# YiwenShaoStephen/mergeNet

Measured on AMD Instinct MI355X. Metric: merged Mpixels/sec at 1024x2048 (speculative fast path; proven path: value_proven_path), higher is better.
Workload: dtype f32

## Files before the change

mergenet_amd/csrc/mergenet_hip.hip:

```cpp
#include <hip/hip_runtime.h>
#include <hip/hip_ext.h>

#include <math.h>
#include <stdio.h>
#include <stdlib.h>
#include <string.h>
#include <time.h>

#include "../../include/mergenet_hip.h"
#include "mn_device.h"
#include "mn_kernels_score.h"
#include "mn_kernels_merge.h"
#include "mn_kernels_finish.h"
#include "mn_kernels_output.h"
#include "mn_kernels_prepare.h"
#include "mn_kernels_cc.h"
#include "mn_kernels_tail.h"
#include "mn_kernels_exact.h"
#include "mn_kernels_reforder.h"

#define MN_NSCALARS 16
#define MN_STAT_BYTES ((((sizeof(Counters) + 15) & ~(size_t)15)) + MN_NSCALARS * sizeof(int) + 4 * sizeof(double))

#define MN_MAX_SUBROUNDS 64
// ... 552 lines not shown
  S.lpvalid = c->lpvalid;
  return S;
}

template <bool FIRST>
static void launch_edge_pass(mn_context* c, const ImgParams& P, hipStream_t st, u64* out, int s) {
  const int* progress = c->progress;
  const dim3 g(grid_for(P.N, 256)), b(256);
  const dim3 gx(8 * ((grid_for(P.N, 256) + 7) / 8));
  const unsigned char* cls0 = c->ocls;
  const unsigned char* matched = c->matched;
  const bool fast = P.omf > 0.0f && P.sdb == 0.0f && !(c->debug_flags & 1);
  if (fast && P.O == 10 && !P.clip)
    hipLaunchKernelGGL((mn_edge_pass_fast<10, FIRST, false>), gx, b, 0, st, P, cls0, matched, out,
                       progress, s);
  else if (fast && P.O == 10)
    hipLaunchKernelGGL((mn_edge_pass_fast<10, FIRST, true>), gx, b, 0, st, P, cls0, matched, out,
                       progress, s);
  else if (fast && P.O == 16 && !P.clip)
    hipLaunchKernelGGL((mn_edge_pass_fast<16, FIRST, false>), gx, b, 0, st, P, cls0, matched, out,
                       progress, s);
  else if (fast && P.O == 16)
    hipLaunchKernelGGL((mn_edge_pass_fast<16, FIRST, true>), gx, b, 0, st, P, cls0, matched, out,
                       progress, s);
  else
    hipLaunchKernelGGL(mn_edge_pass_generic<FIRST>, g, b, 0, st, P, obj_state(c), matched, out, progress, s);
}

static int run_phase_a(mn_context* c, const ImgParams& P, hipStream_t st, bool edge,
                       FillList* fills = nullptr, bool components = false) {
  const int N = P.N;
  FillList own;
  if (!fills) fills = &own;
  if (!components) {
    fills->add(c->lpvalid, N, 0);
    fills->add(c->matched, N, 0);
  }
  fills->launch(st);
  if (components) {
    if (!c->ext_events) MN_HIP(hipEventRecord(c->ev[0], st));
    return MN_OK;
  }
  hipLaunchKernelGGL(mn_init_objects, dim3(grid_for(N, 256)), dim3(256), 0, st, N, c->osize,
                     c->parent, c->mate);
  MN_HIP(hipEventRecord(c->ev[0], st));
  {
    const unsigned blocks = grid_for((size_t)(N >> 2) > 0 ? (size_t)(N >> 2) : 1, 256);
    hipLaunchKernelGGL(mn_class_pass, dim3(blocks), dim3(256), 0, st, P, c->ocls);
  }
  MN_HIP(hipEventRecord(c->ev[1], st));
  if (edge) {
    launch_edge_pass<true>(c, P, st, c->ball, 0);
  }
  MN_HIP(hipEventRecord(c->ev[2], st));
  MN_HIP(hipMemcpyAsync(c->cls0, c->ocls, N, hipMemcpyDeviceToDevice, st));
  MN_HIP(hipGetLastError());
  return MN_OK;
}

static int read_counters(mn_context* c, hipStream_t st) {
  MN_HIP(hipMemcpyAsync(c->h_cnt, c->cnt, sizeof(Counters), hipMemcpyDeviceToHost, st));
  MN_HIP(hipStreamSynchronize(st));
  return MN_OK;
}

static int build_list(mn_context* c, const ImgParams& P, hipStream_t st, size_t cap, RecList L,
                      bool from_pixels, RecList src, int Rsrc, int* Rout, bool fresh_all = false) {
  ObjState S = obj_state(c);
  HashTab T = c->T;
  T.mask = (unsigned)(cap - 1);
  FillList f;
  f.add(T.key, cap * sizeof(u64), 0xFF);
  f.add(T.S, cap * sizeof(i64), 0);
  f.add(T.touched, cap, 0);
  f.add(&c->cnt->n_records, sizeof(int), 0);
  f.add(c->ball, (size_t)P.N * sizeof(u64), 0);
  f.add(c->gmax, 64 * sizeof(unsigned), 0);
  f.launch(st);
  if (from_pixels)
    hipLaunchKernelGGL(mn_build_from_pixels, dim3(grid_for(P.N, 256)), dim3(256), 0, st, P, S, T);
  else
    hipLaunchKernelGGL(mn_rebuild, dim3(grid_for(Rsrc, MN_REBUILD_ITEMS)), dim3(256), 0, st, S, src,
                       Rsrc, (const unsigned char*)c->matched, T, L, c->ball, c->gmax, c->cnt, fresh_all ? 1 : 0);
  if (cap <= (1u << 16))
    hipLaunchKernelGGL(mn_compact<1>, dim3(grid_for(cap, 256)), dim3(256), 0, st, P, S, T, L,
                       c->ball, c->gmax, c->cnt, (const int*)nullptr, (int*)nullptr);
  else
    hipLaunchKernelGGL(mn_compact<4>, dim3(grid_for(cap, MN_COMPACT_SLOTS)), dim3(256), 0, st, P, S, T, L,
                       c->ball, c->gmax, c->cnt, (const int*)nullptr, (int*)nullptr);
  MN_HIP(hipGetLastError());
  if (read_counters(c, st) != MN_OK) return MN_ERR_NO_DEVICE;
  *Rout = c->h_cnt->n_records;
  return MN_OK;
}

static size_t gsum_stride(int N) {
#ifdef MN_GSUM_SKEW
  return ((((size_t)N / 4 + 63) / 64) | 1) * 64;
#else
  return (size_t)N;
#endif
}

template <int PX>
static void launch_cc_px(mn_context* c, const ImgParams& P, hipStream_t st, unsigned kmask, bool hook,
                         bool cls = false, const unsigned* hook_bits = nullptr,
                         hipEvent_t hook_done = nullptr, bool lean_cls = false) {
  const int N = P.N, ngroups = (N + PX - 1) / PX;
  if (!hook) {
    const dim3 g(grid_for(ngroups, MN_CC_SIGN_THREADS)), b(MN_CC_SIGN_THREADS);
    ClsOut CO;
    CO.ocls = lean_cls ? nullptr : c->ocls; CO.cls0 = c->cls0; CO.lpvalid = lean_cls ? nullptr : c->lpvalid;
    CO.gsum = reinterpret_cast<int*>(c->lpsum);
    CO.gstride = gsum_stride(P.N);
    const bool plain = !P.clip && P.sdb == 0.0f;
#define MN_LAUNCH_SIGN(PLAINV, CLSV)                                                                    \
    do {                                                                                                \
      if (c->ext_events)                                                                                \
        hipExtLaunchKernelGGL((mn_cc_sign<PX, PLAINV, (CLSV) && PX == 4>), g, b, 0, st, c->ev[0], c->ev[10], 0, \
                              P, c->cc_bits, c->cc_negbits, c->scalars + 6, c->partial, CO); \
      else                                                                                              \
        hipLaunchKernelGGL((mn_cc_sign<PX, PLAINV, (CLSV) && PX == 4>), g, b, 0, st, P, c->cc_bits, c->cc_negbits, \
                           c->scalars + 6, c->partial, CO);                                             \
    } while (0)
    if (plain && cls) MN_LAUNCH_SIGN(true, true);
    else if (plain) MN_LAUNCH_SIGN(true, false);
    else if (cls) MN_LAUNCH_SIGN(false, true);
    else MN_LAUNCH_SIGN(false, false);
#undef MN_LAUNCH_SIGN
  } else {
    const dim3 gx(8 * ((grid_for(ngroups, 256) + 7) / 8));
    if (hook_done)
      hipExtLaunchKernelGGL(mn_cc_hook<PX>, gx, dim3(256), 0, st, nullptr, hook_done, 0, P,
                            hook_bits ? hook_bits : (const unsigned*)c->cc_bits, c->parent, kmask);
    else
      hipLaunchKernelGGL(mn_cc_hook<PX>, gx, dim3(256), 0, st, P, hook_bits ? hook_bits : (const unsigned*)c->cc_bits,
                         c->parent, kmask);
  }
}

static int run_components(mn_context* c, const ImgParams& P, hipStream_t& st, bool wait, bool with_ball,
                          bool with_compact, bool fork_before_sums, bool cores = false) {
  const int N = P.N;
  ObjState S = obj_state(c);
  const dim3 b(256);
  const bool four = P.W % 4 == 0;
  int kh = -1, kv = -1, dv = 0;
  for (int k = 0; k < P.O; k++) {
    if (kh < 0 && P.di[k] == 0 && P.dj[k] == 1) kh = k;
    if (kv < 0 && P.dj[k] == 0 && (P.di[k] == 1 || P.di[k] == -1)) { kv = k; dv = P.di[k]; }
  }
  const bool few_events = (c->debug_flags & 2) != 0;
  const bool lean = (c->debug_flags & 16) != 0;
  const dim3 tiles((P.W + 63) / 64, (P.H + MN_CC_TILE_ROWS - 1) / MN_CC_TILE_ROWS);
  const bool sweep4 = (N & 3) == 0 && P.W >= 4;
  const size_t sign_blocks = grid_for((size_t)(sweep4 ? N / 4 : N), MN_CC_SIGN_THREADS);
  c->cc_sign_blocks = (int)(sign_blocks * (MN_CC_SIGN_THREADS / 64));
  int* clsmin = c->root;
  int* clsmax = c->mapbuf;
  const bool fused_cls = sweep4;
  const bool lean_cls = fused_cls && !cores;
  if (sweep4) launch_cc_px<4>(c, P, st, 0u, false, fused_cls, nullptr, nullptr, lean_cls);
  else launch_cc_px<1>(c, P, st, 0u, false);
  if (!few_events && !c->ext_events) MN_HIP(hipEventRecord(c->ev[10], st));
  const unsigned* lbits = c->cc_bits;
  unsigned kshort = 0u;
  if (cores) {
    if (!fused_cls) {
      const unsigned blocks = grid_for((size_t)(N >> 2) > 0 ? (size_t)(N >> 2) : 1, 256);
      hipLaunchKernelGGL(mn_class_pass, dim3(blocks), dim3(256), 0, st, P, c->cls0);
    }
    unsigned* bits2 = reinterpret_cast<unsigned*>(c->label);
    for (int k = 0; k < P.O; k++)
      if (c->core_radius < 0 || (abs(P.di[k]) <= c->core_radius && abs(P.dj[k]) <= c->core_radius)) kshort |= 1u << k;
    hipLaunchKernelGGL(mn_core_clean, dim3(grid_for(N, 256)), b, 0, st, P, (const unsigned*)c->cc_bits,
                       (const unsigned char*)c->cls0, c->pruned, kshort);
    hipLaunchKernelGGL(mn_core_bits, dim3(grid_for(N, 256)), b, 0, st, P, (const unsigned char*)c->pruned,
                       (const unsigned*)c->cc_bits, (const unsigned char*)c->cls0, bits2);
    lbits = bits2;
  }
  hipStream_t real = st;
  if (c->replay.capturing) {
    MN_HIP(hipStreamBeginCapture(c->replay.cap, hipStreamCaptureModeThreadLocal));
    st = c->replay.cap;
  }
  unsigned kmask = P.O >= 32 ? 0xFFFFFFFFu : ((1u << P.O) - 1u);
  const bool fork_ext = fork_before_sums && c->ext_events && !c->replay.capturing;
  bool fork_by_hook = false;
  hipLaunchKernelGGL(mn_cc_tiles, tiles, dim3(MN_CC_TILE_ROWS * 64), 0, st, P, lbits, c->parent, kh, kv, dv,
                     c->osize, c->lp_acc, clsmin, clsmax, c->matched);
  if (kh >= 0 || kv >= 0) {
    hipLaunchKernelGGL(mn_cc_borders, tiles, dim3(128), 0, st, P, lbits, c->parent, kh, kv, dv);
    if (kh >= 0) kmask &= ~(1u << kh);
    if (kv >= 0) kmask &= ~(1u << kv);
  }
  hipLaunchKernelGGL(mn_cc_flatten, dim3(grid_for((size_t)(N >> 2) > 0 ? (size_t)(N >> 2) : 1, 256)), b, 0, st, N, c->parent);
  fork_by_hook = fork_ext && kmask;
  if (kmask) {
    if (four) launch_cc_px<4>(c, P, st, kmask, true, false, lbits, fork_by_hook ? c->ev_fork : nullptr);
    else launch_cc_px<1>(c, P, st, kmask, true, false, lbits, fork_by_hook ? c->ev_fork : nullptr);
  }
  if (c->replay.capturing) {
    MN_HIP(hipStreamEndCapture(c->replay.cap, &c->replay.gA));
    MN_HIP(hipGraphInstantiate(&c->replay.eA, c->replay.gA, nullptr, nullptr, 0));
    MN_HIP(hipGraphLaunch(c->replay.eA, real));
    st = real;
  }
  HashTab T = c->T;
  T.mask = (unsigned)(c->cc_cap - 1);
  if (!few_events && !lean) MN_HIP(hipEventRecord(c->ev[7], st));
  if (fork_before_sums) {
    if (!fork_by_hook) MN_HIP(hipEventRecord(c->ev_fork, st));
    MN_HIP(hipStreamWaitEvent(c->side, c->ev_fork, 0));
    st = c->side;
    if (c->replay.capturing) {
      MN_HIP(hipStreamBeginCapture(c->replay.cap, hipStreamCaptureModeThreadLocal));
      st = c->replay.cap;
    }
  }
  if (!few_events && !lean) MN_HIP(hipEventRecord(c->ev[11], st));
  {
    const size_t lds = (size_t)MN_CC_SUM_SLOTS * (P.C + 1) * sizeof(u64);
    if (lds > c->cc_sum_lds) {
      MN_HIP(hipFuncSetAttribute(reinterpret_cast<const void*>(mn_cc_class_sums),
                                 hipFuncAttributeMaxDynamicSharedMemorySize, (int)lds));
      MN_HIP(hipFuncSetAttribute(reinterpret_cast<const void*>(mn_cc_sums),
                                 hipFuncAttributeMaxDynamicSharedMemorySize, (int)lds));
      c->cc_sum_lds = lds;
    }
    const unsigned blocks = grid_for((size_t)(N >> 2) > 0 ? (size_t)(N >> 2) : 1, MN_CC_SUM_THREADS);
    if (fused_cls)
      hipLaunchKernelGGL(mn_cc_sums, dim3((blocks + MN_CC_SUMS_ITERS - 1) / MN_CC_SUMS_ITERS), dim3(MN_CC_SUM_THREADS), lds, st, P, S,
                         (const unsigned char*)c->cls0, (const int*)reinterpret_cast<int*>(c->lpsum), gsum_stride(P.N),
                         c->lp_acc, clsmin, clsmax, cores ? (const unsigned char*)c->pruned : (const unsigned char*)nullptr);
    else
      hipLaunchKernelGGL(mn_cc_class_sums, dim3(blocks), dim3(MN_CC_SUM_THREADS), lds, st, P, S, c->cls0,
                         c->lp_acc, clsmin, clsmax);
  }
  if (!few_events && !lean) MN_HIP(hipEventRecord(c->ev[8], st));
  if (!cores)
  {
    if (sweep4)
      hipLaunchKernelGGL(mn_cc_cross<4>, dim3((unsigned)grid_for((size_t)N / 4, MN_CC_CROSS_THREADS)), dim3(MN_CC_CROSS_THREADS),
                         0, st, P, (const int*)c->parent, T, (const unsigned*)c->cc_negbits, c->scalars + 6, c->cc_tcount);
    else
      hipLaunchKernelGGL(mn_cc_cross<1>, dim3((unsigned)grid_for((size_t)N, MN_CC_CROSS_THREADS)), dim3(MN_CC_CROSS_THREADS),
                         0, st, P, (const int*)c->parent, T, (const unsigned*)c->cc_negbits, c->scalars + 6, c->cc_tcount);
  }
  if (!few_events && !lean) MN_HIP(hipEventRecord(c->ev[9], st));
  hipLaunchKernelGGL(mn_cc_finish, dim3(grid_for((size_t)(N >> 4) > 0 ? (size_t)(N >> 4) : 1, 256)), b, 0, st, P, S,
                     (const unsigned char*)c->matched, (const i64*)c->lp_acc,
                     (const int*)clsmin, (const int*)clsmax, c->mate, cores ? (int*)nullptr : c->cc_roots,
                     c->scalars + 8, c->scalars + 6, lean_cls ? (const unsigned char*)c->cls0 : (const unsigned char*)nullptr);
  if (cores) {
    const unsigned all = P.O >= 32 ? 0xFFFFFFFFu : ((1u << P.O) - 1u);
    if (kshort != all) {
      MN_HIP(hipMemsetAsync(c->matched, 0, (size_t)N, st));
      hipLaunchKernelGGL(mn_core_check, dim3(grid_for(N, 256)), b, 0, st, P, (const int*)c->parent, lbits, c->matched);
      hipLaunchKernelGGL(mn_core_dissolve, dim3(grid_for(N, 256)), b, 0, st, P, S,
                         (const unsigned char*)c->matched, c->scalars + 9);
    }
    hipLaunchKernelGGL(mn_count_cross_edges, dim3(grid_for(N, 256)), b, 0, st, P, (const int*)c->parent, c->touch);
  }
  if (with_compact)
    hipLaunchKernelGGL(mn_compact<4>, dim3(grid_for(c->cc_cap, MN_COMPACT_SLOTS)), dim3(256), 0, st, P, S,
                       T, c->LA, with_ball ? c->ball : (u64*)nullptr, c->gmax, c->cnt,
                       (const int*)c->cc_tcount, c->cc_lcount);
  MN_HIP(hipGetLastError());
  if (!wait) return 0;
  MN_HIP(hipMemcpyAsync(c->h_scalars, c->scalars, MN_NSCALARS * sizeof(int), hipMemcpyDeviceToHost, st));
  MN_HIP(hipMemcpyAsync(c->h_cnt, c->cnt, sizeof(Counters), hipMemcpyDeviceToHost, st));
  MN_HIP(hipStreamSynchronize(st));
  if (c->h_scalars[6] != 0 || c->h_scalars[7] != 0) {
    MN_HIP(hipMemsetAsync(c->cnt, 0, sizeof(Counters), st));
    return 1;
  }
  return 0;
}

static int exact_setup(mn_context* c, const ImgParams& P, hipStream_t st) {
  int rc = x_ensure(c, P.N, P.O, P.C);
  if (rc != MN_OK) return rc;
  mn_context::XWork& w = c->xw;
  XState& X = w.X;
  const size_t N = (size_t)P.N;
  MN_HIP(hipMemsetAsync(X.hs, 0xFF, (size_t)X.nb * 4 * sizeof(XSlot), st));
  MN_HIP(hipMemsetAsync(X.leaf, 0, (((size_t)X.NB << X.Blog) + 1024) * sizeof(unsigned), st));
  MN_HIP(hipMemsetAsync(X.ostamp, 0, (size_t)N * 2 * sizeof(unsigned), st));
  MN_HIP(hipMemsetAsync(X.freeheads, 0xFF, MN_X_FREE_CLASSES * sizeof(unsigned), st));
  memset(w.h_ctl, 0, sizeof(XCtl));
  w.h_ctl->ttrack = getenv("MN_X_NO_TIE_TRACKING") ? 0 : 1;
  w.h_ctl->bump = 0ull;
  MN_HIP(hipMemcpyAsync(X.ctl, w.h_ctl, sizeof(XCtl), hipMemcpyHostToDevice, st));
  hipLaunchKernelGGL(mn_x_init_objects, dim3(grid_for(N, 256)), dim3(256), 0, st, P, X, c->cls0);
  MN_HIP(hipEventRecord(c->ev[1], st));
  hipLaunchKernelGGL(mn_x_init_records, dim3(grid_for((size_t)X.NL, 256)), dim3(256), 0, st, P, X);
  MN_HIP(hipEventRecord(c->ev[2], st));
  MN_HIP(hipGetLastError());
  return MN_OK;
}

static int exact_loop(mn_context** cs, int n, const ImgParams* Ps, hipStream_t st, unsigned char* full) {
  mn_context::XWork& w0 = cs[0]->xw;
  if (w0.batch_cap < n) {
    if (w0.d_P) (void)hipFree(w0.d_P);
    if (w0.d_X) (void)hipFree(w0.d_X);
    w0.d_P = nullptr; w0.d_X = nullptr;
    MN_HIP(hipMalloc(reinterpret_cast<void**>(&w0.d_P), (size_t)n * sizeof(ImgParams)));
    MN_HIP(hipMalloc(reinterpret_cast<void**>(&w0.d_X), (size_t)n * sizeof(XState)));
    w0.batch_cap = n;
  }
  size_t lds = 0;
  long long max_total = 0;
  {
    XState* hx = static_cast<XState*>(malloc((size_t)n * sizeof(XState)));
    if (!hx) return MN_ERR_INTERNAL;
    for (int i = 0; i < n; i++) {
      const XState& X = cs[i]->xw.X;
      hx[i] = X;
      const size_t l = MN_X_LDS_BYTES(X.NBpad);
      if (l > lds) lds = l;
      const long long mt = 8LL * (long long)X.NL + 65536;
      if (mt > max_total) max_total = mt;
    }
    hipError_t e1 = hipMemcpyAsync(w0.d_P, Ps, (size_t)n * sizeof(ImgParams), hipMemcpyHostToDevice, st);
    hipError_t e2 = hipMemcpyAsync(w0.d_X, hx, (size_t)n * sizeof(XState), hipMemcpyHostToDevice, st);
    hipError_t e3 = hipStreamSynchronize(st);
    free(hx);
    MN_HIP(e1); MN_HIP(e2); MN_HIP(e3);
  }
  if (!w0.lds_ready) {
    MN_HIP(hipFuncSetAttribute(reinterpret_cast<const void*>(mn_x_run),
                               hipFuncAttributeMaxDynamicSharedMemorySize, 160 * 1024));
    w0.lds_ready = 1;
  }
  long long per_launch = 1LL << 24;
  if (const char* e = getenv("MN_X_BUDGET")) { const long long v = atoll(e); if (v > 0) per_launch = v; }
  const long long max_launches = 1 << 20;
  for (long long it = 0; it < max_launches; it++) {
    long long most = 0;
    bool any = false;
    for (int i = 0; i < n; i++) {
      mn_context::XWork& w = cs[i]->xw;
      if (it > 0 && w.h_ctl->status != MN_X_BUDGET) continue;
      any = true;
// ... 1491 lines not shown
```

mergenet_amd/csrc/mn_kernels_cc.h:

```cpp
#pragma once

static_assert(MN_MAX_OFFSETS <= 32, "edge masks are 32-bit words: one bit per offset");

#include "mn_device.h"
#include "mn_kernels_merge.h"

#define MN_LP_FIX 16777216.0

__device__ __forceinline__ int mn_cc_find(int* __restrict__ parent, int x) {
  int p = parent[x];
  while (p != x) {
    const int g = parent[p];
    if (g != p) parent[x] = g;
    x = p;
    p = g;
  }
  return x;
}

struct __attribute__((packed, aligned(4))) mn_int4u { int x, y, z, w; };
__device__ __forceinline__ int4 mn_ld_int4_unaligned(const int* __restrict__ p) {
  const mn_int4u t = *reinterpret_cast<const mn_int4u*>(p);
  return make_int4(t.x, t.y, t.z, t.w);
}
// ... 138 lines not shown
          const float x = (PLAIN || first[g] != INT_MIN) ? mn_cc_value<PLAIN>(P, v[g][j]) : 1.0f;
          m[j] |= (x >= P.sep_hi) ? bit : 0u;
          ng[j] |= (x <= P.sep_lo) ? bit : 0u;
          f *= fmaxf(x, 1.0f - x);
        }
      }
    } else {
#pragma unroll
      for (int g = 0; g < G; g++) {
        const unsigned bit = (k0 + g < P.O) ? (1u << ((k0 + g) & 31)) : 0u;
#pragma unroll
        for (int j = 0; j < PX; j++) {
          const bool second = straddle && c0 + j >= P.W;
          const bool inb = ((rin[g] >> (second ? 1 : 0)) & 1) &&
                           (unsigned)(first[g] + j - (second ? P.W : 0)) < (unsigned)P.W;
          const float x = inb ? mn_cc_value<PLAIN>(P, v[g][j]) : 1.0f;
          inmask[j] |= inb ? bit : 0u;
          m[j] |= (x >= P.sep_hi) ? bit : 0u;
          ng[j] |= (x <= P.sep_lo) ? bit : 0u;
          f *= fmaxf(x, 1.0f - x);
        }
      }
    }
    if (((k0 / G) & 3) == 3 || k0 + G >= P.O) {
      t_sum += (double)logf(f);
      f = 1.0f;
    }
  }
  int bad = 0;
#pragma unroll
  for (int j = 0; j < PX; j++) {
    const unsigned in = fast ? rowmask : inmask[j];
    m[j] &= in;
    ng[j] &= in;
    bad += __popc(in & ~(m[j] | ng[j]));
  }
  if (live) {
    if (PX == 4) {
      mn_st_stream(reinterpret_cast<uint4*>(bits + p0), make_uint4(m[0], m[1 % PX], m[2 % PX], m[3 % PX]));
      mn_st_stream(reinterpret_cast<uint4*>(negbits + p0), make_uint4(ng[0], ng[1 % PX], ng[2 % PX], ng[3 % PX]));
    } else {
      bits[p0] = m[0];
      negbits[p0] = ng[0];
    }
  }
  for (int off = 32; off > 0; off >>= 1) {
    bad += __shfl_xor(bad, off);
    t_sum += __shfl_xor(t_sum, off);
  }
  if (lane == 0) {
    if (bad) atomicAdd(violations, bad);
    const size_t waveg = (size_t)blockIdx.x * (MN_CC_SIGN_THREADS / 64) + wave;
    partial[waveg * 2] = t_sum;
    partial[waveg * 2 + 1] = 0.0;
  }
}

__global__ __launch_bounds__(256) void mn_cc_export_neg(ImgParams P, const unsigned* __restrict__ negbits,
                                                        float* __restrict__ out) {
  const int p = blockIdx.x * 256 + threadIdx.x;
  if (p >= P.N) return;
  unsigned left = negbits[p];
  while (left) {
    const int k = __ffs((int)left) - 1;
    left &= left - 1u;
    const float x = mn_same_value(P, P.same[(size_t)k * P.N + p]);
    out[(size_t)k * P.N + p] = logf(x) - mn_log1m(x);
  }
}

#ifndef MN_CC_TILE_ROWS
#define MN_CC_TILE_ROWS 16
#endif
__global__ __launch_bounds__(MN_CC_TILE_ROWS * 64) void mn_cc_tiles(ImgParams P, const unsigned* __restrict__ bits,
                                                    int* __restrict__ parent, int kh, int kv, int dv,
                                                    int* __restrict__ osize, i64* __restrict__ lp_acc,
                                                    int* __restrict__ clsmin, int* __restrict__ clsmax,
                                                    unsigned char* __restrict__ cand) {
  __shared__ int lab[MN_CC_TILE_ROWS * 64];
  const int t = threadIdx.x, lane = t & 63, i = t >> 6;
  const int r = (int)blockIdx.y * MN_CC_TILE_ROWS + i, c = (int)blockIdx.x * 64 + lane;
  const bool in = r < P.H && c < P.W;
  const int p = in ? r * P.W + c : 0;
  const unsigned b = in ? bits[p] : 0u;
  const bool link = kh >= 0 && ((b >> kh) & 1u) && lane < 63;
  const int ni = i + dv;
  const bool vlink = kv >= 0 && ((b >> kv) & 1u) && ni >= 0 && ni < MN_CC_TILE_ROWS;
  const u64 m = __ballot(link);
  const u64 below = lane ? (~m & ((1ull << lane) - 1ull)) : 0ull;
  const int start = below ? (64 - __clzll((long long)below)) : 0;
  lab[t] = i * 64 + start;
  __syncthreads();
  int a = 0, bb = 0;
  bool want = false;
  if (vlink) {
    a = mn_cc_find(lab, t);
    bb = mn_cc_find(lab, ni * 64 + lane);
    want = a != bb;
  }
  u64 todo = __ballot(want);
  const u64 key = mn_key(a, bb);
  while (todo) {
    const int first = __ffsll((long long)todo) - 1;
    const u64 k0v = ((u64)(unsigned)__shfl((int)(key >> 32), first) << 32) |
                    (u64)(unsigned)__shfl((int)(key & 0xFFFFFFFFull), first);
    const bool mine = want && key == k0v;
    if (lane == first) {
      while (a != bb) {
        if (a < bb) { const int x = a; a = bb; bb = x; }
        const int old = atomicMin(&lab[a], bb);
        if (old == a) break;
        a = mn_cc_find(lab, old);
        bb = mn_cc_find(lab, bb);
      }
    }
    todo &= ~__ballot(mine);
  }
  __syncthreads();
  if (!in) return;
  int x = t;
  while (lab[x] != x) x = lab[x];
  parent[p] = ((int)blockIdx.y * MN_CC_TILE_ROWS + (x >> 6)) * P.W + (int)blockIdx.x * 64 + (x & 63);
  cand[p] = (x == t) ? 1 : 0;
  if (x == t) {
    osize[p] = 0;
    for (int c = 0; c < P.C; c++) lp_acc[(size_t)c * P.N + p] = 0;
    clsmin[p] = 255;
    clsmax[p] = 0;
  }
}

__device__ __forceinline__ void mn_cc_wave_union(int* __restrict__ parent, bool want, int a, int b) {
  const int lane = threadIdx.x & 63;
  u64 todo = __ballot(want);
  const u64 key = mn_key(a, b);
  while (todo) {
    const int first = __ffsll((long long)todo) - 1;
    const u64 k0v = ((u64)(unsigned)__shfl((int)(key >> 32), first) << 32) |
                    (u64)(unsigned)__shfl((int)(key & 0xFFFFFFFFull), first);
    const bool mine = want && key == k0v;
    if (lane == first) {
      while (a != b) {
        if (a < b) { const int t = a; a = b; b = t; }
        const int old = atomicMin(&parent[a], b);
        if (old == a) break;
        a = mn_cc_find(parent, old);
        b = mn_cc_find(parent, b);
      }
    }
    todo &= ~__ballot(mine);
  }
}

__global__ __launch_bounds__(128) void mn_cc_borders(ImgParams P, const unsigned* __restrict__ bits,
                                                     int* __restrict__ parent, int kh, int kv, int dv) {
  const int lane = threadIdx.x & 63, wave = threadIdx.x >> 6;
  const int r0 = (int)blockIdx.y * MN_CC_TILE_ROWS, c0 = (int)blockIdx.x * 64;
  int p = -1, q = -1;
  if (wave == 0) {
    const int r = r0 + lane, c = c0 + 63;
    if (kh >= 0 && lane < MN_CC_TILE_ROWS && r < P.H && c + 1 < P.W) {
      p = r * P.W + c;
      if ((bits[p] >> kh) & 1u) q = p + 1;
    }
  } else {
    const int r = dv > 0 ? r0 + MN_CC_TILE_ROWS - 1 : r0, c = c0 + lane;
    if (kv >= 0 && r < P.H && r + dv >= 0 && r + dv < P.H && c < P.W) {
      p = r * P.W + c;
      if ((bits[p] >> kv) & 1u) q = p + dv * P.W;
    }
  }
  int a = 0, b = 0;
  bool want = false;
  if (q >= 0) {
    a = mn_cc_find(parent, p);
    b = mn_cc_find(parent, q);
    want = a != b;
  }
  mn_cc_wave_union(parent, want, a, b);
}

__global__ __launch_bounds__(256) void mn_cc_flatten(int N, int* __restrict__ parent) {
  const int i = blockIdx.x * blockDim.x + threadIdx.x;
  const int n4 = N >> 2;
  if (i < n4) {
    int4 r = *reinterpret_cast<const int4*>(parent + 4 * (size_t)i);
    int4 o = r;
    int x = r.x; while (parent[x] != x) x = parent[x]; o.x = x;
    if (r.y == r.x) o.y = o.x; else { x = r.y; while (parent[x] != x) x = parent[x]; o.y = x; }
    if (r.z == r.x) o.z = o.x; else { x = r.z; while (parent[x] != x) x = parent[x]; o.z = x; }
    if (r.w == r.x) o.w = o.x; else { x = r.w; while (parent[x] != x) x = parent[x]; o.w = x; }
    if (o.x != r.x || o.y != r.y || o.z != r.z || o.w != r.w)
      *reinterpret_cast<int4*>(parent + 4 * (size_t)i) = o;
  }
  if (i < N - (n4 << 2)) {
    const int p = (n4 << 2) + i;
    int x = p; while (parent[x] != x) x = parent[x];
    parent[p] = x;
  }
}

template <int PX>
__global__ __launch_bounds__(256) void mn_cc_hook(ImgParams P, const unsigned* __restrict__ bits,
                                                  int* __restrict__ parent, unsigned kmask) {
  const int ngroups = (P.N + PX - 1) / PX;
  const int tile = mn_xcd_tile((ngroups + 255) >> 8, P.banded);
  const int i = tile < 0 ? ngroups : tile * 256 + threadIdx.x;
  const bool live = i < ngroups;
  const int p0 = live ? PX * i : 0;
  const int r = p0 / P.W, c0 = p0 - r * P.W;
  unsigned b[PX];
  int own[PX];
#pragma unroll
  for (int j = 0; j < PX; j++) { b[j] = 0u; own[j] = 0; }
  if (live) {
    if (PX == 4) {
      const uint4 t = *reinterpret_cast<const uint4*>(bits + p0);
      b[0] = t.x; b[1 % PX] = t.y; b[2 % PX] = t.z; b[3 % PX] = t.w;
      const int4 o = *reinterpret_cast<const int4*>(parent + p0);
      own[0] = o.x; own[1 % PX] = o.y; own[2 % PX] = o.z; own[3 % PX] = o.w;
    } else {
      b[0] = bits[p0];
      own[0] = parent[p0];
    }
  }
  unsigned any = 0u;
#pragma unroll
  for (int j = 0; j < PX; j++) any |= b[j];
  any &= kmask;
  constexpr int G = 4;
  for (int k0 = 0; k0 < P.O; k0 += G) {
    if (__ballot((any >> k0) & ((1u << G) - 1u)) == 0) continue;
    int rq[G][PX];
#pragma unroll
    for (int g = 0; g < G; g++) {
      const int k = k0 + g;
#pragma unroll
      for (int j = 0; j < PX; j++) rq[g][j] = own[j];
      if (k < P.O && ((any >> k) & 1u)) {
        const long long q0 = (long long)(r + P.di[k]) * P.W + c0 + P.dj[k];
        if (PX == 4 && q0 >= 0 && q0 + 3 < P.N) {
          const int4 t = mn_ld_int4_unaligned(parent + q0);
          rq[g][0] = t.x; rq[g][1 % PX] = t.y; rq[g][2 % PX] = t.z; rq[g][3 % PX] = t.w;
        } else {
#pragma unroll
          for (int j = 0; j < PX; j++)
            if (((b[j] >> k) & 1u) && q0 + j >= 0 && q0 + j < P.N) rq[g][j] = parent[q0 + j];
        }
      }
    }
#pragma unroll
    for (int g = 0; g < G; g++) {
      const int k = k0 + g;
      if (k >= P.O) break;
      if (__ballot((any >> k) & 1u) == 0) continue;
#pragma unroll
      for (int j = 0; j < PX; j++) {
        bool want = false;
        int a = 0, bb = 0;
        if (((b[j] & kmask) >> k) & 1u) {
          if (rq[g][j] != own[j]) {
            const int q = p0 + j + P.di[k] * P.W + P.dj[k];
            a = mn_cc_find(parent, p0 + j);
            bb = mn_cc_find(parent, q);
            want = a != bb;
          }
        }
        mn_cc_wave_union(parent, want, a, bb);
      }
    }
  }
}

__global__ __launch_bounds__(256) void mn_core_clean(ImgParams P, const unsigned* __restrict__ bits,
                                                     const unsigned char* __restrict__ cls0,
                                                     unsigned char* __restrict__ clean, unsigned kshort) {
  const int p = blockIdx.x * blockDim.x + threadIdx.x;
  if (p >= P.N) return;
  const int r = p / P.W, c = p - r * P.W;
  const unsigned b = bits[p];
  const unsigned char mine = cls0[p];
  bool ok = true;
  for (int k = 0; k < P.O; k++) {
    if (!((kshort >> k) & 1u)) continue;
    const int di = P.di[k], dj = P.dj[k];
    if (r + di >= 0 && r + di < P.H && c + dj >= 0 && c + dj < P.W) {
      const int q = p + di * P.W + dj;
      ok = ok && ((b >> k) & 1u) && cls0[q] == mine;
    }
    if (r - di >= 0 && r - di < P.H && c - dj >= 0 && c - dj < P.W) {
      const int q = p - di * P.W - dj;
      ok = ok && ((bits[q] >> k) & 1u) && cls0[q] == mine;
    }
  }
  clean[p] = ok ? 1 : 0;
}

__global__ __launch_bounds__(256) void mn_core_bits(ImgParams P, const unsigned char* __restrict__ clean,
                                                    const unsigned* __restrict__ bits,
                                                    const unsigned char* __restrict__ cls0,
                                                    unsigned* __restrict__ bits2) {
  const int p = blockIdx.x * blockDim.x + threadIdx.x;
  if (p >= P.N) return;
  unsigned m = 0u;
  if (clean[p]) {
    const unsigned b = bits[p];
    const unsigned char mine = cls0[p];
    const int r = p / P.W, c = p - r * P.W;
    for (int k = 0; k < P.O; k++) {
      if (!((b >> k) & 1u)) continue;
      const int q = (r + P.di[k]) * P.W + c + P.dj[k];
      if (clean[q] && cls0[q] == mine) m |= 1u << k;
    }
  }
  bits2[p] = m;
}

__global__ __launch_bounds__(256) void mn_core_check(ImgParams P, const int* __restrict__ parent,
                                                     const unsigned* __restrict__ bits2,
// ... 650 lines not shown
```

Before: 16260.

## Add 4-pixel-per-thread CC tile kernel with larger tiles and wave-scan row labels

Adds mn_cc_tiles4, a tile-local connected-components kernel in which each thread handles four consecutive pixels using vector loads and stores. It resolves horizontal runs with a wave ballot/shuffle scan and vertical links with shared-memory union-find. Tiles grow to 32x128 when the width is a multiple of four, and mn_cc_borders is parameterised by tile size so it covers the wider tiles. The goal is less per-pixel work and fewer tile-border unions. The cost is more complex intra-tile logic and larger blocks, which may lower occupancy.

Result: faster. 16590 (median of 6 runs) (+2.0%).

```diff
diff --git a/mergenet_amd/csrc/mergenet_hip.hip b/mergenet_amd/csrc/mergenet_hip.hip
--- a/mergenet_amd/csrc/mergenet_hip.hip
+++ b/mergenet_amd/csrc/mergenet_hip.hip
@@ -728,7 +728,8 @@
   }
   const bool few_events = (c->debug_flags & 2) != 0;
   const bool lean = (c->debug_flags & 16) != 0;
-  const dim3 tiles((P.W + 63) / 64, (P.H + MN_CC_TILE_ROWS - 1) / MN_CC_TILE_ROWS);
+  const int trows = four ? MN_CC_TILE4_ROWS : MN_CC_TILE_ROWS, tcols = four ? MN_CC_TILE4_COLS : 64;
+  const dim3 tiles((P.W + tcols - 1) / tcols, (P.H + trows - 1) / trows);
   const bool sweep4 = (N & 3) == 0 && P.W >= 4;
   const size_t sign_blocks = grid_for((size_t)(sweep4 ? N / 4 : N), MN_CC_SIGN_THREADS);
   c->cc_sign_blocks = (int)(sign_blocks * (MN_CC_SIGN_THREADS / 64));
@@ -763,10 +764,14 @@
   unsigned kmask = P.O >= 32 ? 0xFFFFFFFFu : ((1u << P.O) - 1u);
   const bool fork_ext = fork_before_sums && c->ext_events && !c->replay.capturing;
   bool fork_by_hook = false;
-  hipLaunchKernelGGL(mn_cc_tiles, tiles, dim3(MN_CC_TILE_ROWS * 64), 0, st, P, lbits, c->parent, kh, kv, dv,
-                     c->osize, c->lp_acc, clsmin, clsmax, c->matched);
+  if (four)
+    hipLaunchKernelGGL((mn_cc_tiles4<MN_CC_TILE4_ROWS, MN_CC_TILE4_COLS>), tiles, dim3(MN_CC_TILE4_ROWS * MN_CC_TILE4_COLS / 4),
+                       0, st, P, lbits, c->parent, kh, kv, dv, c->osize, c->lp_acc, clsmin, clsmax, c->matched);
+  else
+    hipLaunchKernelGGL(mn_cc_tiles, tiles, dim3(MN_CC_TILE_ROWS * 64), 0, st, P, lbits, c->parent, kh, kv, dv,
+                       c->osize, c->lp_acc, clsmin, clsmax, c->matched);
   if (kh >= 0 || kv >= 0) {
-    hipLaunchKernelGGL(mn_cc_borders, tiles, dim3(128), 0, st, P, lbits, c->parent, kh, kv, dv);
+    hipLaunchKernelGGL(mn_cc_borders, tiles, dim3(64 + tcols), 0, st, P, lbits, c->parent, kh, kv, dv, trows, tcols);
     if (kh >= 0) kmask &= ~(1u << kh);
     if (kv >= 0) kmask &= ~(1u << kv);
   }
diff --git a/mergenet_amd/csrc/mn_kernels_cc.h b/mergenet_amd/csrc/mn_kernels_cc.h
--- a/mergenet_amd/csrc/mn_kernels_cc.h
+++ b/mergenet_amd/csrc/mn_kernels_cc.h
@@ -314,19 +314,108 @@
   }
 }
 
-__global__ __launch_bounds__(128) void mn_cc_borders(ImgParams P, const unsigned* __restrict__ bits,
-                                                     int* __restrict__ parent, int kh, int kv, int dv) {
+#ifndef MN_CC_TILE4_ROWS
+#define MN_CC_TILE4_ROWS 32
+#endif
+#ifndef MN_CC_TILE4_COLS
+#define MN_CC_TILE4_COLS 128
+#endif
+static_assert(MN_CC_TILE4_ROWS <= 64 && MN_CC_TILE4_COLS <= 128 && MN_CC_TILE_ROWS <= 64,
+              "mn_cc_borders covers at most 64 tile rows and 128 tile columns");
+static_assert(MN_CC_TILE4_ROWS * MN_CC_TILE4_COLS / 4 <= 1024, "a tile of mn_cc_tiles4 is one block");
+template <int TR, int TC>
+__global__ __launch_bounds__(TR * TC / 4) void mn_cc_tiles4(ImgParams P, const unsigned* __restrict__ bits,
+                                                    int* __restrict__ parent, int kh, int kv, int dv,
+                                                    int* __restrict__ osize, i64* __restrict__ lp_acc,
+                                                    int* __restrict__ clsmin, int* __restrict__ clsmax,
+                                                    unsigned char* __restrict__ cand) {
+  constexpr int LPR = TC / 4;
+  static_assert(LPR == 16 || LPR == 32 || LPR == 64, "a wave holds whole tile rows");
+  __shared__ __attribute__((aligned(16))) int lab[TR * TC];
+  const int t = threadIdx.x, lane = t & 63;
+  const int i = t / LPR, l = t % LPR;
+  const int r = (int)blockIdx.y * TR + i, c = (int)blockIdx.x * TC + 4 * l;
+  const bool in = r < P.H && c < P.W;
+  const int p = in ? r * P.W + c : 0;
+  unsigned b[4] = {0u, 0u, 0u, 0u};
+  if (in) {
+    const uint4 v = *reinterpret_cast<const uint4*>(bits + p);
+    b[0] = v.x; b[1] = v.y; b[2] = v.z; b[3] = v.w;
+  }
+  const bool h0 = kh >= 0 && ((b[0] >> kh) & 1u), h1 = kh >= 0 && ((b[1] >> kh) & 1u);
+  const bool h2 = kh >= 0 && ((b[2] >> kh) & 1u);
+  const bool h3 = kh >= 0 && ((b[3] >> kh) & 1u) && l < LPR - 1;
+  const u64 m3 = __ballot(h3);
+  const bool k0 = !(l > 0 && ((m3 >> (lane - 1)) & 1ull));
+  const bool k1 = !h0, k2 = !h1, k3 = !h2;
+  const int last = k3 ? 3 : k2 ? 2 : k1 ? 1 : k0 ? 0 : -1;
+  const u64 anyk = __ballot(last >= 0);
+  const int seg = lane - l;
+  const u64 below = anyk & ((1ull << lane) - 1ull) & ~((1ull << seg) - 1ull);
+  const int src = below ? 63 - __clzll((long long)below) : lane;
+  const int lsrc = __shfl(last, src);
+  const int s0 = k0 ? 4 * l : 4 * (src - seg) + lsrc;
+  const int s1 = k1 ? 4 * l + 1 : s0, s2 = k2 ? 4 * l + 2 : s1, s3 = k3 ? 4 * l + 3 : s2;
+  *reinterpret_cast<int4*>(lab + 4 * t) = make_int4(i * TC + s0, i * TC + s1, i * TC + s2, i * TC + s3);
+  const int ni = i + dv;
+  const bool vok = kv >= 0 && ni >= 0 && ni < TR;
+  __syncthreads();
+#pragma unroll
+  for (int j = 0; j < 4; j++) {
+    int a = 0, bb = 0;
+    bool want = false;
+    if (vok && ((b[j] >> kv) & 1u)) {
+      a = mn_cc_find(lab, 4 * t + j);
+      bb = mn_cc_find(lab, ni * TC + 4 * l + j);
+      want = a != bb;
+    }
+    mn_cc_wave_union(lab, want, a, bb);
+  }
+  __syncthreads();
+  if (!in) return;
+  int x[4];
+  const int4 lv = *reinterpret_cast<const int4*>(lab + 4 * t);
+  const int l4[4] = {lv.x, lv.y, lv.z, lv.w};
+#pragma unroll
+  for (int j = 0; j < 4; j++) {
+    if (j > 0 && l4[j] == l4[j - 1]) { x[j] = x[j - 1]; continue; }
+    int y = l4[j];
+    if (y != 4 * t + j) { int z = lab[y]; while (z != y) { y = z; z = lab[y]; } }
+    x[j] = y;
+  }
+  const int g0 = (int)blockIdx.y * TR * P.W + (int)blockIdx.x * TC;
+  int gid[4];
+#pragma unroll
+  for (int j = 0; j < 4; j++) gid[j] = g0 + (x[j] / TC) * P.W + (x[j] % TC);
+  *reinterpret_cast<int4*>(parent + p) = make_int4(gid[0], gid[1], gid[2], gid[3]);
+  uchar4 cd;
+  cd.x = x[0] == 4 * t; cd.y = x[1] == 4 * t + 1; cd.z = x[2] == 4 * t + 2; cd.w = x[3] == 4 * t + 3;
+  *reinterpret_cast<uchar4*>(cand + p) = cd;
+#pragma unroll
+  for (int j = 0; j < 4; j++) {
+    if (x[j] == 4 * t + j) {
+      osize[p + j] = 0;
+      for (int cc = 0; cc < P.C; cc++) lp_acc[(size_t)cc * P.N + p + j] = 0;
+      clsmin[p + j] = 255;
+      clsmax[p + j] = 0;
+    }
+  }
+}
+
+__global__ __launch_bounds__(192) void mn_cc_borders(ImgParams P, const unsigned* __restrict__ bits,
+                                                     int* __restrict__ parent, int kh, int kv, int dv,
+                                                     int trows, int tcols) {
   const int lane = threadIdx.x & 63, wave = threadIdx.x >> 6;
-  const int r0 = (int)blockIdx.y * MN_CC_TILE_ROWS, c0 = (int)blockIdx.x * 64;
+  const int r0 = (int)blockIdx.y * trows, c0 = (int)blockIdx.x * tcols;
   int p = -1, q = -1;
   if (wave == 0) {
-    const int r = r0 + lane, c = c0 + 63;
-    if (kh >= 0 && lane < MN_CC_TILE_ROWS && r < P.H && c + 1 < P.W) {
+    const int r = r0 + lane, c = c0 + tcols - 1;
+    if (kh >= 0 && lane < trows && r < P.H && c + 1 < P.W) {
       p = r * P.W + c;
       if ((bits[p] >> kh) & 1u) q = p + 1;
     }
   } else {
-    const int r = dv > 0 ? r0 + MN_CC_TILE_ROWS - 1 : r0, c = c0 + lane;
+    const int r = dv > 0 ? r0 + trows - 1 : r0, c = c0 + (int)threadIdx.x - 64;
     if (kv >= 0 && r < P.H && r + dv >= 0 && r + dv < P.H && c < P.W) {
       p = r * P.W + c;
       if ((bits[p] >> kv) & 1u) q = p + dv * P.W;
```
